# Mahdi-Si/VAE-TEB

Hardware: AMD Instinct MI355X
Metric: train samples/sec + ELBO, 4096-pt windows, batch 256, 1/2/4/8 MI355X (higher is better)
Workload: dtype bf16 MFMA (decoder heads + conv blocks + ResidualMLP linears, LSTM recurrences f16 fwd / bf16 bwd), fp32 accumulation; fp32 LayerNorm / BatchNorm / LSTM state / front-end / optimizer

## Files before the change

include/vaeteb.h:

```cpp
#ifndef VAETEB_H
#define VAETEB_H

#include <stdint.h>

#ifdef __cplusplus
extern "C" {
#endif

#define VT_OK 0
#define VT_ERR_ARG (-1)
#define VT_ERR_LAYOUT (-2)
#define VT_ERR_HIP (-3)

#define VT_FFT_MAX_LDS 8192

const char* vt_last_error(void);
int vt_stream_fork(void* from, void* to);
int vt_stream_mark(void* stream, int* slot);
int vt_stream_wait_mark(void* stream, int slot);
int vt_abi_version(void);
int vt_arrive_reset(void* stream);
int vt_capture_info(void* stream, char* buf, int len);
int vt_set_h16_format(int fp16);
int vt_get_h16_format(void);


int vt_fe_spectrum(const float* x, int64_t rows, int N, int n_pad, int pad_left, int pad_mode, const void* tw,
                   void* xhat, void* stream);

int vt_fe_lowpass(const float* x, int64_t rows, int64_t x_row_stride, int N, int n_pad, int pad_left,
                  const float* h0, int radius, int step, int start, int S, float* out, int64_t out_row_stride,
                  void* stream);

int vt_fe_wavelet(const void* xhat, int64_t B, int C, int n_pad, const float* psi, int n_items, const int* items,
                  const void* tw, int N, int pad_left, void* analytic, int n_slots, const float* h0, int radius,
                  int step, int start, int S, float* s1, int s1_channels, void* stream);

int vt_fe_pairs(const void* analytic, int64_t B, int n_slots, int N, int n_pad, int pad_left, int n_pairs,
                const int* slot_i, const int* slot_j, const float* power, const void* tw, const float* phi0, int dec,
                int start, int S, int pad_mode, float* out, void* stream);

int vt_fe_set_pairs_persist(int grid);
int vt_fe_set_pairs_direct(int on);
int vt_fe_set_pairs_half(int on);
int vt_fe_set_analytic_polar(int on);

int vt_fe_set_pairs_stamps(void* buf);

int vt_fe_normalize(const float* in, int64_t B, int C, int in_C, int S, const int* kind, const float* mean, const float* stdv,
                    float log_eps, float* out, int out_C, int out_off, void* stream);
int vt_fe_normalize_window(const float* in, int64_t B, int C, int in_C, int in_S, int s0, int S_len,
                           const int* kind, const float* mean, const float* stdv, float log_eps, float* out,
                           int out_C, int out_off, void* stream);
int vt_copy_cols(const float* src, int64_t rows, int ld_src, int src_col0, int ncols, float* dst, int ld_dst,
                 int dst_col0, void* stream);
int vt_clamp_bwd(const float* g, const float* x, int64_t n, float lo, float hi, float* gx, void* stream);
int vt_zero_ranges(float* base, int n, const int64_t* starts, const int64_t* ends, void* stream);
int vt_normalize_raw(const float* x, int64_t rows, int64_t row_stride, int N, float mean, float stdv, float* out,
                     void* stream);

#define VT_STATS_CHUNK_ROWS 32
#define VT_STATS_CHUNK_COLS 1024
int vt_stats_chunking(int* rows, int* cols);
int vt_stats_workspace_bytes(int64_t B, int C, int S_len, int64_t* bytes);
int vt_stats_accum(const float* in, int64_t B, int C, int in_C, int in_S, int s0, int S_len, const int* kind,
                   double log_eps, int64_t* count, double* sum, double* sum_sq, void* work, int64_t work_bytes,
                   void* stream);
int vt_stats_accum_raw(const float* x, int64_t rows, int64_t row_stride, int N, int64_t* count, double* sum,
                       double* sum_sq, void* work, int64_t work_bytes, void* stream);

int vt_fft(const void* in, void* out, int64_t rows, int n, int inverse, const void* tw, int tw_stride,
           void* stream);
int vt_fft_large(const void* in, void* out, void* ws, int64_t rows, int n, int inverse, const void* tw,
                 void* stream);
int vt_cdgmm(const void* A, const void* B, int b_is_real, void* C, int64_t rows, int n, void* stream);
int vt_scat_filter_sub(const void* A, int B, int64_t a_rows, int n, const int* a_idx, const float* pool,
                       const int64_t* f_off, int P, int k, void* out, void* stream);
int vt_scat_mod_spec(const void* A, int B, int64_t a_rows, int n, const int* a_idx, const float* pool,
                     const int64_t* f_off, int P, int k, const void* tw, void* out, void* stream);
int vt_scat_lowpass(const void* U, int B, int P, int n, const float* phi, int k, int i0, int i1, const int* ch,
                    int out_C, const void* tw, float* out, void* stream);
int vt_modulus_cplx(const void* in, void* out, int64_t count, void* stream);
int vt_modulus(const void* in, float* out, int64_t count, void* stream);
int vt_modulus_bwd(const void* in, const float* mod, const float* grad, void* grad_in, int64_t count, void* stream);
int vt_subsample_fourier(const void* in, void* out, int64_t rows, int n, int k, void* stream);
int vt_pad_reflect(const float* in, float* out, int64_t rows, int N, int pad_left, int pad_right, void* stream);


int vt_elbo_workspace_floats(void);

int vt_elbo_latent_fwd(const float* mu_c, const float* lv_q, const float* mu_y, const float* lv_p, const float* eps,
                       int64_t rows, int D, float* z, float* mu_post, float* kl, float* ws, void* stream);
int vt_elbo_latent_bwd(const float* mu_c, const float* lv_q, const float* mu_y, const float* lv_p, const float* eps,
                       int64_t rows, int D, const float* g_z, const float* g_mu_post, const float* g_kl,
                       float* g_mu_c, float* g_lv_q, float* g_mu_y, float* g_lv_p, void* stream);
int vt_elbo_output_fwd(const float* mu, const float* lv, const float* y, int64_t n_nll, const float* lin,
                       const float* t_st, const float* t_ph, int64_t rows, int c_st, int c_ph, float* g_mu,
                       float* g_lv, float* g_lin, float* nll, float* mse, float* ws, void* stream);
int vt_scale_by_device_scalar(float* x, int64_t n, const float* s, void* stream);

int vt_grad_norm_workspace_floats(void);
int vt_grad_norm_clip(const float* g, int64_t n, float pre_scale, float max_norm, float* out2, float* ws,
                      void* stream);
int vt_grad_norm_clip_scaled(const float* g, int64_t n, float pre_scale, float max_norm, float* out3, float* ws,
                             float* scaler, float growth_factor, float backoff_factor, int growth_interval,
                             void* stream);
int vt_adamw_step(float* p, const float* g, float* m, float* v, int64_t n, float lr, float beta1, float beta2,
                  float eps, float weight_decay, int step, const float* gscale, void* stream);
int vt_adamw_step_dev(float* p, const float* g, float* m, float* v, int64_t n, float lr, float beta1, float beta2,
                      float eps, float weight_decay, int* step, float* coef, const float* gscale, void* stream);
int vt_adamw_step_dev_shadow(float* p, const float* g, float* m, float* v, int64_t n, float lr, float beta1,
                             float beta2, float eps, float weight_decay, int* step, float* coef, const float* gscale,
                             int n_tiled, const int64_t* tiled_off, const int* tiled_N, const int* tiled_K,
                             const int64_t* tiled_w16, const int64_t* tiled_w16t, void* stream);
int vt_adamw_step_dev_skip(float* p, const float* g, float* m, float* v, int64_t n, float lr, float beta1,
                           float beta2, float eps, float weight_decay, int* step, float* coef, const float* gscale,
                           const float* skip, void* stream);
int vt_adamw_step_dev_shadow_skip(float* p, const float* g, float* m, float* v, int64_t n, float lr, float beta1,
                                  float beta2, float eps, float weight_decay, int* step, float* coef,
                                  const float* gscale, int n_tiled, const int64_t* tiled_off, const int* tiled_N,
                                  const int* tiled_K, const int64_t* tiled_w16, const int64_t* tiled_w16t,
                                  const float* skip, void* stream);
int vt_adamw_set_vector(int on);
int vt_cast_bf16(const float* src, void* dst, int64_t n, void* stream);
int vt_cast_bf16_to_f32(const void* src, float* dst, int64_t n, void* stream);

int vt_gemm_splits_hint(int64_t M, int N, int64_t K);
int vt_linear_fwd(const float* X, int64_t R, int K, const float* W, int N, const float* bias, float* Y, void* stream);
int vt_linear_bwd_data(const float* dY, int64_t R, int N, const float* W, int K, float* dX, int accumulate,
                       void* stream);
int vt_linear_bwd_weight(const float* dY, int64_t R, int N, const float* X, int K, float* dW, float* db,
                         int accumulate, float* ws, int64_t ws_floats, void* stream);
int vt_linear_ln_fwd(const float* X, int64_t R, int K, const float* W, int N, const float* bias, const float* gamma,
                     const float* beta, int act, float eps, float* Y, float* xhat, float* rstd, void* stream);
int vt_colsum(const float* X, int64_t R, int N, float* out, int accumulate, float* ws, int64_t ws_floats,
              void* stream);

#define VT_MLP_MAX_LAYERS 34
#define VT_MLP_MAX_WIDTH 144
int vt_resmlp_sizes(int n_layers, const int* dims, const int* layer_ln, const int* layer_act, int skip,
                    int64_t rows, int64_t* sizes);
int vt_resmlp_fwd(int n_layers, const int* dims, const int* layer_ln, const int* layer_act, int skip, float eps,
                  const float* const* params, const float* x, int64_t rows, float* out, float* xhat, float* rstd,
                  void* stream);
int vt_resmlp_bwd(int n_layers, const int* dims, const int* layer_ln, const int* layer_act, int skip, float eps,
                  const float* const* params, const float* dout, const float* xhat, const float* rstd, int64_t rows,
                  float* dx, float* const* grads, int accumulate, float* ws, int64_t ws_floats, void* stream);

int vt_resmlp_bf16_sizes(int n_layers, const int* dims, const int* layer_ln, const int* layer_act, int skip,
                         int64_t rows, int64_t* sizes);
int vt_resmlp_bf16_fwd(int n_layers, const int* dims, const int* layer_ln, const int* layer_act, int skip, float eps,
                       const float* const* params, const float* x, int64_t rows, float* out, float* xhat, float* rstd,
                       void* stream);
int vt_resmlp_bf16_bwd(int n_layers, const int* dims, const int* layer_ln, const int* layer_act, int skip, float eps,
                       const float* const* params, const float* dout, const float* xhat, const float* rstd,
                       int64_t rows, float* dx, float* const* grads, int accumulate, float* ws, int64_t ws_floats,
                       void* stream);
int vt_resmlp_bf16_plan(int n_layers, const int* dims, const int* layer_ln, const int* layer_act, int skip, float eps,
                        const float* const* params, int64_t rows, int64_t* handle, void* stream);
int vt_resmlp_bf16_prep_batch(int n, const int64_t* handles, void* stream);
int vt_resmlp_bf16_fwd_prepped(int n_layers, const int* dims, const int* layer_ln, const int* layer_act, int skip,
                               float eps, const float* const* params, const float* x, int64_t rows, float* out,
                               float* xhat, float* rstd, void* stream);
int vt_resmlp_bf16_split_sizes(int n_layers, const int* dims, const int* layer_ln, const int* layer_act, int skip,
                               int64_t rows, int64_t* sizes);
int vt_resmlp_bf16_bwd_data(int n_layers, const int* dims, const int* layer_ln, const int* layer_act, int skip,
                            float eps, const float* const* params, const float* dout, const float* xhat,
                            const float* rstd, int64_t rows, float* dx, float* const* grads, int accumulate,
                            void* dz16, float* ws, int64_t ws_floats, void* stream);
int vt_resmlp_bf16_bwd_weight(int n_layers, const int* dims, const int* layer_ln, const int* layer_act, int skip,
                              float eps, const float* const* params, const float* xhat, const void* dz16,
                              int64_t rows, float* const* grads, int accumulate, float* ws, int64_t ws_floats,
                              void* stream);
int vt_resmlp_bf16_set_stamps(void* buf);

int vt_mfma_supported(int K, int N);
int vt_mfma_workspace_floats(int64_t R, int K, int N, int64_t* floats);
int vt_mfma_weight_shadow(const float* W, int N, int K, void* W16, void* W16t, void* stream);
int vt_mfma_linear_fwd(const float* X, int64_t R, int K, const void* W16, int N, const float* bias, float* Y,
                       float* ws, int64_t ws_floats, void* stream);
int vt_mfma_linear_bwd_data(const float* dY, int64_t R, int N, const void* W16t, int K, float* dX, int accumulate,
                            float* ws, int64_t ws_floats, void* stream);
int vt_mfma_linear_bwd_weight(const float* dY, int64_t R, int N, const float* X, int K, float* dW, float* db,
                              int accumulate, float* ws, int64_t ws_floats, void* stream);

int vt_conv1d_out_len(int L_in, int K, int mode, int up);
int vt_conv1d_fwd(const float* X, int B, int L_in, int Cin, const float* W, int Cout, int K, int mode, int up,
                  float* Y, void* stream);
int vt_conv1d_bwd_data(const float* dY, int B, int L_in, int Cin, const float* W, int Cout, int K, int mode, int up,
                       float* dX, int accumulate, float* gpad, void* stream);
int vt_conv1d_bwd_weight(const float* dY, const float* X, int B, int L_in, int Cin, int Cout, int K, int mode, int up,
                         float* dW, int accumulate, float* ws, int64_t ws_floats, void* stream);
int vt_conv1d_bn_workspace_floats(int B, int L_in, int Cin, int Cout, int K, int mode, int up, int64_t* floats);
int vt_conv1d_bn_fwd(const float* X, int B, int L_in, int Cin, const float* W, int Cout, int K, int mode, int up,
                     const float* gamma, const float* beta, int act, float eps, float momentum, float* conv_out,
                     float* Y, float* mean, float* rstd, float* run_mean, float* run_var, float* ws,
                     int64_t ws_floats, void* stream);
int vt_conv1d_bf16_shadow(const float* W, int Cout, int Cin, int K, void* w16, void* w16t, void* stream);
int vt_conv1d_bf16_shadow_batch(int n, const int64_t* W, const int* Cout, const int* Cin, const int* K,
                                const int64_t* w16, const int64_t* w16t, void* stream);
int vt_conv_bf16_set_staging(int mode);
int vt_conv_bf16_set_kernels(int flags);
int vt_conv1d_bn_fwd_bf16(const float* X, int B, int L_in, int Cin, const void* w16, int Cout, int K, int mode,
                          int up, const float* gamma, const float* beta, int act, float eps, float momentum,
                          float* conv_out, float* Y, float* mean, float* rstd, float* run_mean, float* run_var,
                          float* ws, int64_t ws_floats, void* stream);
int vt_conv1d_bn_fwd_bf16_in(const float* X, const float* in_mean, const float* in_rstd, const float* in_gamma,
                             const float* in_beta, int in_act, int B, int L_in, int Cin, const void* w16, int Cout,
                             int K, int mode, int up, const float* gamma, const float* beta, int act, float eps,
                             float momentum, float* conv_out, float* Y, float* mean, float* rstd, float* run_mean,
                             float* run_var, float* ws, int64_t ws_floats, void* stream);
int vt_conv1d_fwd_bf16(const float* X, int B, int L_in, int Cin, const void* w16, int Cout, int K, int mode, int up,
                       float* Y, void* stream);
int vt_conv1d_bwd_gpad_bf16(const float* dY, int B, int L_in, int Cin, const void* w16t, int Cout, int K, int mode,
                            int up, float* gpad, void* stream);
int vt_conv1d_bwd_weight_bf16(const float* dY, const float* X, int B, int L_in, int Cin, int Cout, int K, int mode,
                              int up, float* dW, int accumulate, float* ws, int64_t ws_floats, void* stream);
int vt_conv1d_bwd_gpad_bf16_bn(const float* dY, const float* Xc, const float* bnp, int act, int64_t M, int B,
                               int L_in, int Cin, const void* w16t, int Cout, int K, int mode, int up, float* gpad,
                               void* dxbn16, void* stream);
int vt_conv1d_bwd_dx_bf16_bn(const float* dY, const float* Xc, const float* bnp, int act, int64_t M, int B, int L_in,
                             int Cin, const void* w16t, int Cout, int K, int mode, int up, float* dX, float* edge,
                             void* dxbn16, void* stream);
int vt_conv1d_bwd_weight_bf16_dy16(const void* dY16, const float* X, int B, int L_in, int Cin, int Cout, int K,
                                   int mode, int up, float* dW, int accumulate, float* ws, int64_t ws_floats,
                                   void* stream);
int vt_conv1d_bwd_weight_bf16_dy16s(const void* dY16, int dys, const float* X, int B, int L_in, int Cin, int Cout,
                                    int K, int mode, int up, float* dW, int accumulate, float* ws, int64_t ws_floats,
                                    void* stream);
int vt_conv1d_bwd_weight_bf16_in(const float* dY, const void* dY16, int dys, const float* X, const float* in_mean,
                                 const float* in_rstd, const float* in_gamma, const float* in_beta, int in_act, int B,
                                 int L_in, int Cin, int Cout, int K, int mode, int up, float* dW, int accumulate,
                                 float* ws, int64_t ws_floats, void* stream);
int vt_batchnorm_bwd_x16(const float* dY, const float* Xc, const float* bnp, int act, int64_t M, int C, void* d16,
                         void* stream);
int vt_conv1d_bwd_dx16(const void* d16, int B, int L_in, int Cin, const void* w16t, int Cout, int K, int mode, int up,
                       float* dX, float* edge, void* stream);
int vt_conv1d_direct_fwd(const float* X, int B, int L_in, int Cin, const float* W, int Cout, int K, int mode, int up,
                         float* Y, void* stream);
int vt_conv1d_direct_bwd_gpad(const float* dY, int B, int L_in, int Cin, const float* W, int Cout, int K, int mode,
                              int up, float* gpad, void* stream);
int vt_conv1d_fold(const float* gpad, int B, int L_in, int Cin, int Cout, int K, int mode, int up, float* dX,
                   int accumulate, void* stream);
int vt_conv1d_direct_bwd_weight(const float* dY, const float* X, int B, int L_in, int Cin, int Cout, int K, int mode,
                                int up, float* dW, int accumulate, float* ws, int64_t ws_floats, void* stream);

int vt_layernorm_fwd(const float* x, int64_t R, int C, const float* gamma, const float* beta, int act, float eps,
                     float* y, float* xhat, float* rstd, void* stream);
int vt_layernorm_bwd(const float* dy, const float* xhat, const float* rstd, int64_t R, int C, const float* gamma,
                     const float* beta, int act, float* dx, float* dgamma, float* dbeta, int accumulate_params,
                     float* ws, int64_t ws_floats, void* stream);
int vt_batchnorm_fwd(const float* x, int64_t M, int C, const float* gamma, const float* beta, int act, float eps,
                     float momentum, float* y, float* mean, float* rstd, float* run_mean, float* run_var, float* ws,
                     int64_t ws_floats, void* stream);
int vt_batchnorm_bwd(const float* dy, const float* x, int64_t M, int C, const float* mean, const float* rstd,
                     const float* gamma, const float* beta, int act, float* dx, float* dgamma, float* dbeta,
                     int accumulate_params, float* ws, int64_t ws_floats, void* stream);
int vt_batchnorm_fwd_dropout(const float* x, int64_t M, int C, const float* gamma, const float* beta, int act,
                             float eps, float momentum, float* y, float* mean, float* rstd, float* run_mean,
                             float* run_var, int L, float p, int64_t seed, const void* seed_offset, float* ws,
                             int64_t ws_floats, void* stream);
int vt_batchnorm_bwd_dropout(const float* dy, const float* x, int64_t M, int C, const float* mean, const float* rstd,
                             const float* gamma, const float* beta, int act, int L, float p, int64_t seed,
                             const void* seed_offset, float* dx, float* dgamma, float* dbeta, int accumulate_params,
                             float* ws, int64_t ws_floats, void* stream);
int vt_batchnorm_bwd_coef(const float* dy, const float* x, int64_t M, int C, const float* mean, const float* rstd,
                          const float* gamma, const float* beta, int act, float* dgamma, float* dbeta,
                          int accumulate_params, float* bnp, float* ws, int64_t ws_floats, void* stream);
int vt_batchnorm_eval(const float* x, int64_t M, int C, const float* run_mean, const float* run_var, float eps,
                      const float* gamma, const float* beta, int act, float* y, void* stream);
int vt_syncbn_sums(const float* x, const float* dy, int64_t M, int C, int which, const float* mean,
                   const float* rstd, const float* gamma, const float* beta, int act, double* sums, float* ws,
                   int64_t ws_floats, void* stream);
int vt_syncbn_stats(const double* sums, int C, int which, float eps, float momentum, float* mean, float* rstd,
                    float* run_mean, float* run_var, float* dgamma, float* dbeta, int accumulate, void* stream);
int vt_batchnorm_apply(const float* x, int64_t M, int C, const float* mean, const float* rstd, const float* gamma,
                       const float* beta, int act, float* y, void* stream);
int vt_syncbn_bwd_dx(const float* dy, const float* x, int64_t M, int C, const float* mean, const float* rstd,
                     const float* gamma, const float* beta, int act, const double* sums, float* dx, float* ws,
                     void* stream);
int vt_act_fwd(const float* x, int64_t n, int act, float* y, void* stream);
int vt_act_bwd(const float* dy, const float* x, int64_t n, int act, float* dx, void* stream);

int vt_lstm_layer_fwd(const float* gin, const float* w_hh, const float* b_hh, int B, int S, int hidden, float* out_h,
                      float* out_hprev, float* out_c, float* gates, void* stream);
int vt_lstm_layer_bwd(const float* dh_out, const float* gates, const float* cst, const float* w_hh, int B, int S,
                      int hidden, float* dgates, void* stream);
int vt_lstm_layer_fwd_x(const float* x, int In, const float* w_ih, const float* b_ih, const float* w_hh,
                        const float* b_hh, int B, int S, int hidden, float* out_h, float* out_hprev, float* out_c,
                        float* gates, void* stream);
int vt_lstm_layer_bwd_x(const float* dh_out, const float* gates, const float* cst, const float* w_hh,
                        const float* w_ih, int In, int B, int S, int hidden, float* dgates, float* dx, void* stream);
int vt_lstm16_layer_fwd(const float* x, int In, const float* w_ih, const float* b_ih, const float* w_hh,
                        const float* b_hh, int B, int S, int hidden, float* out_h, float* out_hprev, float* out_c,
                        float* gates, void* stream);
int vt_lstm16_layer_bwd(const float* dh_out, const float* gates, const float* cst, const float* w_hh,
                        const float* w_ih, int In, int B, int S, int hidden, float* dgates, float* dx, void* stream);
int vt_lstm16_pair_fwd(const float* x, int In, const float* w_ih0, const float* b_ih0, const float* w_hh0,
                       const float* b_hh0, const float* w_ih1, const float* b_ih1, const float* w_hh1,
                       const float* b_hh1, int B, int seq, int hidden, float* h0, float* c0, float* gates0, float* h1,
                       float* c1, float* gates1, void* stream);
int vt_lstm16_pair_bwd(const float* dh_out, const float* gates1, const float* c1, const float* w_hh1,
                       const float* w_ih1, const float* gates0, const float* c0, const float* w_hh0,
                       const float* w_ih0, int In0, int B, int seq, int hidden, void* dgates1, void* dgates0,
                       float* dx, void* stream, int dg_bf16);
int vt_lstm16_quad_fwd(const float* x, int In, const float* const* params, int B, int seq, int hidden,
                       float* const* outs, void* stream);
int vt_lstm16_quad_bwd(const float* dh_out, const float* const* w, const float* const* gc, int In0, int B, int seq,
                       int hidden, void* const* dg, float* dmid, float* dx, void* stream, int dg_bf16);
int vt_lstm16_chain_errors(int* count, int reset);
int vt_lstm_layer_bwd_weight(const float* dgates, const float* x, int In, const float* hprev, int B, int S,
                             int hidden, float* dw_ih, float* dw_hh, float* db_ih, float* db_hh, int accumulate,
                             float* ws, int64_t ws_floats, void* stream);
int vt_lstm16_layer_bwd_weight(const float* dgates, const float* x, int In, const float* h, int B, int S,
                               int hidden, float* dw_ih, float* dw_hh, float* db_ih, float* db_hh, int accumulate,
                               float* ws, int64_t ws_floats, void* stream);
int vt_lstm16_dg16_ok(int In);
int vt_lstm16_bwd_weight_multi(int nl, const void* const* dgates, const int* dg_bf16, const float* const* x,
                               const int* In, const float* const* h, int B, int seq, int hidden, float* const* grads,
                               const int* accumulate, float* ws, int64_t ws_floats, void* stream);

int vt_zconv_fwd(const float* X, int ldx, int B, int L, int Cin, const float* W, int Cout, int K, int pad_left,
                 float* Y, int ldy, int accumulate, void* stream);
int vt_zconv_bwd_data(const float* dY, int ldy, int B, int L, int Cin, const float* W, int Cout, int K, int pad_left,
                      float* dX, int ldx, int accumulate, void* stream);
int vt_zconv16_ws_floats(int Cin, int Cout, int K, int64_t* floats);
int vt_zconv16_fwd(const float* X, int ldx, int B, int L, int Cin, const float* W, int Cout, int K, int pad_left,
                   float* Y, int ldy, int accumulate, float* ws, int64_t ws_floats, void* stream);
int vt_zconv16_bwd_data(const float* dY, int ldy, int B, int L, int Cin, const float* W, int Cout, int K, int pad_left,
                        float* dX, int ldx, int accumulate, float* ws, int64_t ws_floats, void* stream);
int vt_zconv16_taps_elems(int Cin, int Cout, int K, int64_t* elems);
int vt_zconv16_taps(int n, const int64_t* W, const int* Cin, const int* Cout, const int* K, int flip,
                    const int64_t* T, void* stream);
int vt_zconv16_fwd_t(const float* X, int ldx, int B, int L, int Cin, const void* T, int Cout, int K, int pad_left,
                     float* Y, int ldy, int accumulate, void* stream);
int vt_zconv16_bwd_data_t(const float* dY, int ldy, int B, int L, int Cin, const void* T, int Cout, int K,
                          int pad_left, float* dX, int ldx, int accumulate, void* stream);
int vt_zconv16_bwd_weight(const float* dY, int ldy, const float* X, int ldx, int B, int L, int Cin, int Cout, int K,
                          int pad_left, float* dW, int accumulate, float* ws, int64_t ws_floats, void* stream);
int vt_zconv_bwd_weight_ws_floats(int B, int Cin, int Cout, int K, int64_t* floats);
int vt_zconv_bwd_weight(const float* dY, int ldy, const float* X, int ldx, int B, int L, int Cin, int Cout, int K,
                        int pad_left, float* dW, int accumulate, float* ws, int64_t ws_floats, void* stream);
int vt_maxpool3_fwd(const float* X, int B, int L, int C, float* Y, void* stream);
int vt_maxpool3_bwd(const float* dY, const float* X, int B, int L, int C, float* dX, int accumulate, void* stream);
int vt_add_act_fwd(const float* A, const float* Bm, int64_t n, int act, float* Y, void* stream);
int vt_add_act_dropout_fwd(const float* A, const float* Bm, int64_t n, int C, int act, int L, float p, int64_t seed,
                           const void* seed_offset, float* S_out, float* Y, void* stream);
int vt_act_dropout_bwd(const float* dY, const float* S_in, int64_t n, int C, int act, int L, float p, int64_t seed,
                       const void* seed_offset, float* dX, void* stream);
int vt_dropout_apply(const float* X, int64_t n, int C, int L, float p, int64_t seed, const void* seed_offset, float* Y,
                     void* stream);
int vt_dropout_seed_advance(void* offset, void* stream);
int vt_time_mean_fwd(const float* X, int B, int L, int C, float* Y, void* stream);
int vt_time_mean_bwd(const float* dY, int B, int L, int C, float* dX, int accumulate, void* stream);
int vt_attn_fwd(const float* qkv, int B, int S, int H, float scale, float p, int64_t seed, const void* seed_offset,
                float* out, float* lse, void* stream);
int vt_attn_bwd(const float* qkv, const float* out, const float* dout, const float* lse, int B, int S, int H,
                float scale, float p, int64_t seed, const void* seed_offset, float* dqkv, void* stream);
int vt_cross_entropy_fwd(const float* logits, const int64_t* labels, int B, int C, float* loss, float* probs,
                         void* stream);
int vt_cross_entropy_bwd(const float* probs, const int64_t* labels, int B, int C, const float* g, float* dlogits,
                         void* stream);

int vt_stepgraph_build(void* graph, int n_streams, void** handle);
int vt_stepgraph_launch(void* handle, void* const* streams);
int vt_stepgraph_info(void* handle, int* n_kernel, int* n_memcpy, int* n_memset, int* n_waits);
int vt_stepgraph_destroy(void* handle);
int vt_bucket_marker(int bucket, void* stream);
int vt_stepgraph_markers(void* handle, int* n_ops, int* n_markers, int* ends, int* buckets, int cap);
int vt_stepgraph_launch_range(void* handle, void* const* streams, int begin, int end, int flags);

#ifdef __cplusplus
}
#endif
#endif
```

vae-teb_amd/csrc/mfma.hip:

```cpp
#include "h16.h"

namespace vt {

constexpr int QM = 256, QN = 64, QK = 64, QT = 512;
constexpr int ROWB = QK * 2;
constexpr int A_BYTES = QM * ROWB;
constexpr int B_BYTES = QN * ROWB;
constexpr int NA = 3, NB = 8;
constexpr int GEMM_LDS = NA * A_BYTES + NB * B_BYTES;

__device__ __forceinline__ int swz(int r, int c) { return c ^ ((r >> 1) & 7); }

__device__ __forceinline__ void glds16(const void* src, char* lds) {
    __builtin_amdgcn_global_load_lds((const __attribute__((address_space(1))) void*)src,
                                     (__attribute__((address_space(3))) void*)lds, 16, 0, 0);
}

VT_ARRIVE_POOL(g_arrive_gemm);

typedef unsigned u32x4 __attribute__((ext_vector_type(4)));
__device__ __forceinline__ void st_agent4(__amdgpu_buffer_rsrc_t r, unsigned off, f32x4 v) {
    __builtin_amdgcn_raw_buffer_store_b128(__builtin_bit_cast(u32x4, v), r, (int)off, 0, CPOL_SC1);
}
__device__ __forceinline__ f32x4 ld_agent4(__amdgpu_buffer_rsrc_t r, unsigned off) {
    return __builtin_bit_cast(f32x4, __builtin_amdgcn_raw_buffer_load_b128(r, (int)off, 0, CPOL_SC1));
}

__device__ __forceinline__ bool last_arrival_in(unsigned* ctr, unsigned total, unsigned* flag) {
    asm volatile("s_waitcnt vmcnt(0)" ::: "memory");
    __syncthreads();
    if (threadIdx.x == 0) {
        const unsigned old = atomicAdd(ctr, 1u);
        const bool last = old == total - 1;
        if (last) atomicExch(ctr, 0u);
        *flag = last ? 1u : 0u;
    }
    __syncthreads();
    return *flag != 0u;
}

template <typename H>
__global__ __launch_bounds__(QT) void k_mfma_gemm(const H* __restrict__ A, int64_t lda,
                                                  const H* __restrict__ B, int64_t ldb, int M, int N, int K,
                                                  float* __restrict__ C, int64_t ldc, const float* __restrict__ bias,
                                                  int accumulate, float* __restrict__ part, unsigned slot0) {
    extern __shared__ __attribute__((aligned(16))) char smem[];
    char* sa = smem;
    char* sb = smem + NA * A_BYTES;
    const int tid = threadIdx.x, lane = tid & 63, w = tid >> 6;
    const int n0 = blockIdx.x * QN, m0 = blockIdx.y * QM;
    const int64_t kbeg = (int64_t)blockIdx.z * K;
    const int T = K / QK;

    const int rsub = lane >> 3, pos = lane & 7;
    auto kof = [&](int t) { return kbeg + (int64_t)(t < T ? t : T - 1) * QK; };
    auto issue_a = [&](int t) {
        const int64_t k0 = kof(t);
        char* st = sa + (t % NA) * A_BYTES;
#pragma unroll
        for (int i = 0; i < 4; ++i) {
            const int r = 32 * w + 8 * i + rsub;
            glds16(A + (int64_t)(m0 + r) * lda + k0 + 8 * swz(r, pos), st + (32 * w + 8 * i) * ROWB);
        }
    };
    auto issue_b = [&](int t) {
        const int64_t k0 = kof(t);
        const int r = 8 * w + rsub;
        glds16(B + (int64_t)(n0 + r) * ldb + k0 + 8 * swz(r, pos), sb + (t % NB) * B_BYTES + 8 * w * ROWB);
    };

    f32x4 acc[2][4];
#pragma unroll
    for (int i = 0; i < 2; ++i)
#pragma unroll
        for (int j = 0; j < 4; ++j) acc[i][j] = f32x4{0.f, 0.f, 0.f, 0.f};

    const int lr = lane & 15, lc = lane >> 4;
    auto compute = [&](int t) {
        const char* ta = sa + (t % NA) * A_BYTES;
        const char* tb = sb + (t % NB) * B_BYTES;
#pragma unroll
        for (int h = 0; h < 2; ++h) {
            const int c = 4 * h + lc;
            hv8<H> af[2], bfr[4];
#pragma unroll
            for (int i = 0; i < 2; ++i) {
                const int r = 32 * w + 16 * i + lr;
                af[i] = *(const hv8<H>*)(ta + r * ROWB + 16 * swz(r, c));
            }
#pragma unroll
            for (int j = 0; j < 4; ++j) {
                const int r = 16 * j + lr;
                bfr[j] = *(const hv8<H>*)(tb + r * ROWB + 16 * swz(r, c));
            }
#pragma unroll
            for (int i = 0; i < 2; ++i)
#pragma unroll
                for (int j = 0; j < 4; ++j)
                    acc[i][j] = mfma16(af[i], bfr[j], acc[i][j]);
        }
    };

#pragma unroll
    for (int t = 0; t < NB - 1; ++t) issue_b(t);
    issue_a(0);
    issue_a(1);
    for (int t = 0; t < T; ++t) {
        if (t == 0) asm volatile("s_waitcnt vmcnt(4)" ::: "memory");
        else if (t == 1) asm volatile("s_waitcnt vmcnt(5)" ::: "memory");
        else asm volatile("s_waitcnt vmcnt(6)" ::: "memory");
        asm volatile("s_waitcnt lgkmcnt(0)" ::: "memory");
        __builtin_amdgcn_s_barrier();
        issue_a(t + 2);
        issue_b(t + NB - 1);
        compute(t);
    }
    asm volatile("s_waitcnt vmcnt(0)" ::: "memory");

    if (part) {
        const int splits = gridDim.z, z = blockIdx.z;
        const unsigned tile = blockIdx.y * gridDim.x + blockIdx.x;
        const int64_t slab = (int64_t)QT * 32 * 4;
        const __amdgpu_buffer_rsrc_t pr = agent_rsrc(part + (int64_t)tile * splits * QT * 32, splits * slab);
#pragma unroll
        for (int g = 0; g < 8; ++g) st_agent4(pr, (unsigned)(z * slab + (g * QT + tid) * 16), acc[g >> 2][g & 3]);
        if (!last_arrival_in(&g_arrive_gemm[slot0 + tile], (unsigned)splits, (unsigned*)smem)) return;
#pragma unroll
        for (int g = 0; g < 8; ++g) {
            f32x4 s = z == 0 ? acc[g >> 2][g & 3] : ld_agent4(pr, (unsigned)((g * QT + tid) * 16));
            for (int p = 1; p < splits; ++p)
                s += p == z ? acc[g >> 2][g & 3] : ld_agent4(pr, (unsigned)(p * slab + (g * QT + tid) * 16));
            acc[g >> 2][g & 3] = s;
        }
    }
#pragma unroll
    for (int i = 0; i < 2; ++i)
#pragma unroll
        for (int j = 0; j < 4; ++j) {
            const int col = n0 + 16 * j + lr;
            const float bcol = bias ? bias[col] : 0.f;
#pragma unroll
            for (int r = 0; r < 4; ++r) {
                const int row = m0 + 32 * w + 16 * i + 4 * lc + r;
                if (row >= M) continue;
                float o = acc[i][j][r] + bcol;
                if (accumulate) o = C[(int64_t)row * ldc + col] + o;
                C[(int64_t)row * ldc + col] = o;
            }
        }
}

template <typename H>
__global__ void k_bf16_rows(const float* __restrict__ X, int64_t M, int K, H* __restrict__ out, int64_t Mpad,
                            int Kpad) {
    const int64_t i = (int64_t)blockIdx.x * blockDim.x + threadIdx.x;
    const int64_t total = Mpad * Kpad;
    if (i >= total) return;
    const int64_t m = i / Kpad;
    const int k = (int)(i - m * Kpad);
    out[i] = (m < M && k < K) ? (H)X[m * K + k] : (H)0.f;
}

template <typename H>
__global__ __launch_bounds__(256) void k_bf16_transpose(const float* __restrict__ X, int64_t R, int Cn,
                                                        H* __restrict__ out, int64_t Cpad, int64_t Rpad) {
    __shared__ float tile[64][65];
    const int64_t r0 = (int64_t)blockIdx.x * 64, c0 = (int64_t)blockIdx.y * 64;
    const int tx = threadIdx.x & 63, ty = threadIdx.x >> 6;
    for (int i = ty; i < 64; i += 4) {
        const int64_t r = r0 + i, c = c0 + tx;
        tile[i][tx] = (r < R && c < Cn) ? X[r * Cn + c] : 0.f;
    }
    __syncthreads();
    for (int i = ty; i < 64; i += 4) {
        const int64_t c = c0 + i, r = r0 + tx;
        if (c < Cpad && r < Rpad) out[c * Rpad + r] = (H)tile[tx][i];
    }
}

template <typename H>
__global__ __launch_bounds__(256) void k_bf16_shadow(const float* __restrict__ W, int N, int K,
                                                     H* __restrict__ W16, H* __restrict__ W16t) {
    __shared__ float tile[64][65];
    const int64_t n0 = (int64_t)blockIdx.y * 64, k0 = (int64_t)blockIdx.x * 64;
    const int tx = threadIdx.x & 63, ty = threadIdx.x >> 6;
    for (int i = ty; i < 64; i += 4) {
        const float v = W[(n0 + i) * K + k0 + tx];
        tile[i][tx] = v;
        W16[(n0 + i) * K + k0 + tx] = (H)v;
    }
    __syncthreads();
    for (int i = ty; i < 64; i += 4) W16t[(k0 + i) * N + n0 + tx] = (H)tile[tx][i];
}

typedef short v4i16 __attribute__((ext_vector_type(4)));
typedef short v8i16 __attribute__((ext_vector_type(8)));
constexpr int DWT = 128, DWC = 64;
constexpr int DWS = DWT + 16;
constexpr int DWIMG = DWC * DWS + (DWC / 8) * 64;

__device__ __forceinline__ int dw_pos(int r, int c) { return r * DWS + (r >> 3) * 64 + c; }

template <typename H>
__device__ __forceinline__ hv8<H> dw_frag(const H* img, int row0, int col0) {
    const int lane = threadIdx.x & 63, g = lane >> 4, q = (lane >> 2) & 3, p = lane & 3;
    const H* a0 = img + dw_pos(row0 + 8 * g + q, col0 + 4 * p);
    const H* a1 = img + dw_pos(row0 + 8 * g + q + 4, col0 + 4 * p);
    const v4i16 lo = __builtin_amdgcn_ds_read_tr16_b64_v4i16((__attribute__((address_space(3))) v4i16*)a0);
    const v4i16 hi = __builtin_amdgcn_ds_read_tr16_b64_v4i16((__attribute__((address_space(3))) v4i16*)a1);
    const v8i16 r = __builtin_shufflevector(lo, hi, 0, 1, 2, 3, 4, 5, 6, 7);
    return __builtin_bit_cast(hv8<H>, r);
}

template <typename H>
__global__ __launch_bounds__(256) void k_mfma_dw(const float* __restrict__ dY, int64_t R, int N,
                                                 const float* __restrict__ X, int K, float* __restrict__ dW,
                                                 int accumulate) {
    __shared__ __attribute__((aligned(16))) H img[2][DWIMG];
    const int tid = threadIdx.x, lane = tid & 63, w = tid >> 6, wm = w >> 1, wn = w & 1;
    const int n0 = blockIdx.y * DWT, k0 = blockIdx.x * DWT;
    float4 pf[2][8];
    auto load = [&](int64_t r0) {
#pragma unroll
        for (int i = 0; i < 8; ++i) {
            const int e = tid + 256 * i, row = e >> 5, q4 = e & 31;
            const bool ok = r0 + row < R;
            pf[0][i] = ok ? *(const float4*)(dY + (r0 + row) * N + n0 + 4 * q4) : make_float4(0.f, 0.f, 0.f, 0.f);
            pf[1][i] = ok ? *(const float4*)(X + (r0 + row) * K + k0 + 4 * q4) : make_float4(0.f, 0.f, 0.f, 0.f);
        }
    };
    auto store = [&]() {
#pragma unroll
        for (int o = 0; o < 2; ++o)
#pragma unroll
            for (int i = 0; i < 8; ++i) {
                const int e = tid + 256 * i, row = e >> 5, q4 = e & 31;
                const hv4<H> v = {(H)pf[o][i].x, (H)pf[o][i].y, (H)pf[o][i].z, (H)pf[o][i].w};
                *(hv4<H>*)(img[o] + dw_pos(row, 4 * q4)) = v;
            }
    };
    f32x4 acc[4][4];
#pragma unroll
    for (int i = 0; i < 4; ++i)
#pragma unroll
        for (int j = 0; j < 4; ++j) acc[i][j] = f32x4{0.f, 0.f, 0.f, 0.f};
    load(0);
    for (int64_t r0 = 0; r0 < R; r0 += DWC) {
        store();
        __syncthreads();
        if (r0 + DWC < R) load(r0 + DWC);
#pragma unroll
        for (int s = 0; s < DWC / 32; ++s) {
            hv8<H> a[4], b[4];
#pragma unroll
            for (int i = 0; i < 4; ++i) a[i] = dw_frag(img[0], 32 * s, 64 * wm + 16 * i);
#pragma unroll
            for (int j = 0; j < 4; ++j) b[j] = dw_frag(img[1], 32 * s, 64 * wn + 16 * j);
#pragma unroll
            for (int i = 0; i < 4; ++i)
#pragma unroll
                for (int j = 0; j < 4; ++j)
                    acc[i][j] = mfma16(a[i], b[j], acc[i][j]);
        }
        __syncthreads();
    }
    const int lr = lane & 15, lc = lane >> 4;
    float* c0 = dW + (int64_t)(n0 + 64 * wm + 4 * lc) * K + k0 + 64 * wn + lr;
    if (accumulate) {
        f32x4 old[4][4];
#pragma unroll
        for (int i = 0; i < 4; ++i)
#pragma unroll
            for (int j = 0; j < 4; ++j)
#pragma unroll
                for (int rr = 0; rr < 4; ++rr) old[i][j][rr] = c0[(int64_t)(16 * i + rr) * K + 16 * j];
#pragma unroll
        for (int i = 0; i < 4; ++i)
#pragma unroll
            for (int j = 0; j < 4; ++j) acc[i][j] += old[i][j];
    }
#pragma unroll
    for (int i = 0; i < 4; ++i)
#pragma unroll
        for (int j = 0; j < 4; ++j)
#pragma unroll
            for (int rr = 0; rr < 4; ++rr) c0[(int64_t)(16 * i + rr) * K + 16 * j] = acc[i][j][rr];
}

static inline int64_t up_to(int64_t x, int64_t m) { return (x + m - 1) / m * m; }

static int mfma_splits(int64_t tiles, int64_t ktiles) {
    int best = 1;
    for (int64_t d = 1; d <= ktiles && d <= 64; ++d)
        if (ktiles % d == 0 && tiles * d <= 320) best = (int)d;
    return best;
}

struct MfmaPlan {
    int64_t Mpad, Kpad, a_floats, part_floats;
    int splits;
};

static MfmaPlan plan(int64_t M, int N, int64_t K) {
    MfmaPlan p;
    p.Mpad = up_to(M, QM);
    p.Kpad = up_to(K, QK);
    p.a_floats = up_to(p.Mpad * p.Kpad / 2, 64);
    p.splits = mfma_splits((p.Mpad / QM) * (N / QN), p.Kpad / QK);
    p.part_floats = p.splits > 1 ? (int64_t)p.splits * p.Mpad * N : 0;
    return p;
}

template <typename H>
static int run(const char* who, const H* A, const H* B, int64_t ldb, int64_t M, int N, const MfmaPlan& p,
               float* C, const float* bias, int accumulate, float* part, hipStream_t st) {
    static bool attr = false;
    if (!attr) {
        if (hipFuncSetAttribute((const void*)k_mfma_gemm<H>, hipFuncAttributeMaxDynamicSharedMemorySize, GEMM_LDS) !=
            hipSuccess) {
            set_error("%s: cannot allow %d B of LDS for k_mfma_gemm", who, GEMM_LDS);
            return VT_ERR_HIP;
        }
        attr = true;
    }
    const int kper = (int)(p.Kpad / p.splits);
    dim3 grid(N / QN, (unsigned)(p.Mpad / QM), p.splits);
    const unsigned tiles = grid.x * grid.y;
    hipLaunchKernelGGL(k_mfma_gemm<H>, grid, dim3(QT), GEMM_LDS, st, A, p.Kpad, B, ldb, (int)M, N, kper, C, (int64_t)N,
                       bias, accumulate, p.splits > 1 ? part : nullptr, p.splits > 1 ? arrive_slots(tiles, st) : 0u);
    VT_LAUNCH_CHECK(who);
    return VT_OK;
}

}

using namespace vt;

extern "C" {

int vt_mfma_supported(int K, int N) { return (K > 0 && N > 0 && K % QK == 0 && N % QN == 0) ? 1 : 0; }

int vt_mfma_workspace_floats(int64_t R, int K, int N, int64_t* floats) {
    VT_CHECK_ARG(R > 0 && K > 0 && N > 0 && floats, "vt_mfma_workspace_floats: shape");
    MfmaPlan f = plan(R, N, K), d = plan(R, K, N), w = plan(N, K, R);
    const int64_t wf = w.a_floats + up_to((int64_t)K * w.Kpad / 2, 64) + w.part_floats + N;
    int64_t m = f.a_floats + f.part_floats;
    if (d.a_floats + d.part_floats > m) m = d.a_floats + d.part_floats;
    if (wf > m) m = wf;
    *floats = m;
    return VT_OK;
}

int vt_mfma_weight_shadow(const float* W, int N, int K, void* W16, void* W16t, void* stream) {
    VT_CHECK_ARG(vt_mfma_supported(K, N) && W && W16 && W16t, "vt_mfma_weight_shadow: K and N must be multiples of 64");
    VT_H16(hipLaunchKernelGGL(k_bf16_shadow<H>, dim3(K / 64, N / 64), dim3(256), 0, S(stream), W, N, K, (H*)W16,
                              (H*)W16t));
    VT_LAUNCH_CHECK("vt_mfma_weight_shadow");
    return VT_OK;
}

int vt_mfma_linear_fwd(const float* X, int64_t R, int K, const void* W16, int N, const float* bias, float* Y,
                       float* ws, int64_t ws_floats, void* stream) {
    VT_CHECK_ARG(R > 0 && vt_mfma_supported(K, N), "vt_mfma_linear_fwd: K and N must be positive multiples of 64");
    MfmaPlan p = plan(R, N, K);
    VT_CHECK_ARG(p.a_floats + p.part_floats <= ws_floats, "vt_mfma_linear_fwd: workspace too small");
    const int64_t tot = p.Mpad * p.Kpad;
    int rc = VT_OK;
    VT_H16(H* A = (H*)ws;
           hipLaunchKernelGGL(k_bf16_rows<H>, dim3((unsigned)((tot + 255) / 256)), dim3(256), 0, S(stream), X, R, K, A,
                              p.Mpad, (int)p.Kpad);
           rc = run("vt_mfma_linear_fwd", (const H*)A, (const H*)W16, K, R, N, p, Y, bias, 0, ws + p.a_floats,
                    S(stream)));
    return rc;
}

int vt_mfma_linear_bwd_data(const float* dY, int64_t R, int N, const void* W16t, int K, float* dX, int accumulate,
                            float* ws, int64_t ws_floats, void* stream) {
    VT_CHECK_ARG(R > 0 && vt_mfma_supported(N, K), "vt_mfma_linear_bwd_data: K and N must be positive multiples of 64");
    MfmaPlan p = plan(R, K, N);
    VT_CHECK_ARG(p.a_floats + p.part_floats <= ws_floats, "vt_mfma_linear_bwd_data: workspace too small");
    const int64_t tot = p.Mpad * p.Kpad;
    int rc = VT_OK;
    VT_H16(H* A = (H*)ws;
           hipLaunchKernelGGL(k_bf16_rows<H>, dim3((unsigned)((tot + 255) / 256)), dim3(256), 0, S(stream), dY, R, N, A,
                              p.Mpad, (int)p.Kpad);
           rc = run("vt_mfma_linear_bwd_data", (const H*)A, (const H*)W16t, N, R, K, p, dX, nullptr, accumulate,
                    ws + p.a_floats, S(stream)));
    return rc;
}

int vt_mfma_linear_bwd_weight(const float* dY, int64_t R, int N, const float* X, int K, float* dW, float* db,
                              int accumulate, float* ws, int64_t ws_floats, void* stream) {
    VT_CHECK_ARG(R > 0 && vt_mfma_supported(K, N), "vt_mfma_linear_bwd_weight: K and N must be positive multiples of 64");
    if (N % DWT == 0 && K % DWT == 0) {
        VT_H16(hipLaunchKernelGGL(k_mfma_dw<H>, dim3(K / DWT, N / DWT), dim3(256), 0, S(stream), dY, R, N, X, K, dW,
                                  accumulate));
        VT_LAUNCH_CHECK("vt_mfma_linear_bwd_weight");
        return db ? vt_colsum(dY, R, N, db, accumulate, ws, ws_floats, stream) : VT_OK;
    }
    MfmaPlan p = plan(N, K, R);
    const int64_t b_floats = up_to((int64_t)K * p.Kpad / 2, 64);
    VT_CHECK_ARG(p.a_floats + b_floats + p.part_floats + N <= ws_floats, "vt_mfma_linear_bwd_weight: workspace too small");
    float* part = ws + p.a_floats + b_floats;
    int rc = VT_OK;
    VT_H16(H* A = (H*)ws;
           H* Bt = (H*)(ws + p.a_floats);
           hipLaunchKernelGGL(k_bf16_transpose<H>, dim3((unsigned)(p.Kpad / 64), (unsigned)(p.Mpad / 64)), dim3(256), 0,
                              S(stream), dY, R, N, A, p.Mpad, p.Kpad);
           hipLaunchKernelGGL(k_bf16_transpose<H>, dim3((unsigned)(p.Kpad / 64), (unsigned)(K / 64)), dim3(256), 0,
                              S(stream), X, R, K, Bt, (int64_t)K, p.Kpad);
           rc = run("vt_mfma_linear_bwd_weight", (const H*)A, (const H*)Bt, p.Kpad, N, K, p, dW, nullptr, accumulate,
                    part, S(stream)));
    if (rc || !db) return rc;
    return vt_colsum(dY, R, N, db, accumulate, part, ws_floats - p.a_floats - b_floats, stream);
}

}
```

Before: 33830.

## Add in-workgroup split-K MFMA GEMM for linear forward and backward-data

Adds a new GEMM kernel in which the four wave pairs of a 512-thread workgroup each handle one quarter of K on a 64x64 output tile. The partial sums are then reduced through LDS and written with the bias, instead of using the old 256-row tile with grid-level split-K partial buffers. The planner selects it by default for forward and data-gradient linears when padded K is a multiple of 256. The aim is more workgroups for small-M or skinny GEMMs and no extra partial-sum global traffic or reduction pass. A toggle restores the old grid-split path.

```diff
diff --git a/include/vaeteb.h b/include/vaeteb.h
--- a/include/vaeteb.h
+++ b/include/vaeteb.h
@@ -183,6 +183,7 @@
                             float* ws, int64_t ws_floats, void* stream);
 int vt_mfma_linear_bwd_weight(const float* dY, int64_t R, int N, const float* X, int K, float* dW, float* db,
                               int accumulate, float* ws, int64_t ws_floats, void* stream);
+int vt_mfma_set_grid_split(int on);
 
 int vt_conv1d_out_len(int L_in, int K, int mode, int up);
 int vt_conv1d_fwd(const float* X, int B, int L_in, int Cin, const float* W, int Cout, int K, int mode, int up,
diff --git a/vae-teb_amd/csrc/mfma.hip b/vae-teb_amd/csrc/mfma.hip
--- a/vae-teb_amd/csrc/mfma.hip
+++ b/vae-teb_amd/csrc/mfma.hip
@@ -150,6 +150,126 @@
         }
 }
 
+constexpr int WM = 64;
+constexpr int WQ_BYTES = WM * ROWB;
+constexpr int W_STAGE = 4 * WQ_BYTES;
+constexpr int WNA = 2, WNB = 3;
+constexpr int WG_LDS = (WNA + WNB) * W_STAGE;
+constexpr int WP_ROW = QN + 4;
+static_assert(WNA == 2 && WNB >= WNA, "k_mfma_gemm_wg: the vmcnt derivation assumes A one tile ahead, B at least as far");
+static_assert(WG_LDS <= 160 * 1024 && 4 * WM * WP_ROW * 4 <= WG_LDS, "k_mfma_gemm_wg: LDS budget");
+
+template <typename H>
+__global__ __launch_bounds__(QT) void k_mfma_gemm_wg(const H* __restrict__ A, int64_t lda,
+                                                     const H* __restrict__ B, int64_t ldb, int M, int N, int K,
+                                                     float* __restrict__ C, int64_t ldc,
+                                                     const float* __restrict__ bias, int accumulate) {
+    extern __shared__ __attribute__((aligned(16))) char smem[];
+    char* sa = smem;
+    char* sb = smem + WNA * W_STAGE;
+    const int tid = threadIdx.x, lane = tid & 63, w = tid >> 6, q = w >> 1, hm = w & 1;
+    const int n0 = blockIdx.x * QN, m0 = blockIdx.y * WM;
+    const int64_t kbeg = (int64_t)q * K;
+    const int T = K / QK;
+
+    const int rsub = lane >> 3, pos = lane & 7;
+    auto issue = [&](const H* src, int64_t ld, int row0, char* stages, int nst, int t) {
+        if (t < 0 || t >= T) return;
+        const int64_t k0 = kbeg + (int64_t)t * QK;
+        char* st = stages + (t % nst) * W_STAGE + q * WQ_BYTES;
+#pragma unroll
+        for (int i = 0; i < 4; ++i) {
+            const int r = 32 * hm + 8 * i + rsub;
+            glds16(src + (int64_t)(row0 + r) * ld + k0 + 8 * swz(r, pos), st + (32 * hm + 8 * i) * ROWB);
+        }
+    };
+    auto issue_a = [&](int t) { issue(A, lda, m0, sa, WNA, t); };
+    auto issue_b = [&](int t) { issue(B, ldb, n0, sb, WNB, t); };
+
+    f32x4 acc[2][4];
+#pragma unroll
+    for (int i = 0; i < 2; ++i)
+#pragma unroll
+        for (int j = 0; j < 4; ++j) acc[i][j] = f32x4{0.f, 0.f, 0.f, 0.f};
+
+    const int lr = lane & 15, lc = lane >> 4;
+    auto compute = [&](int t) {
+        const char* ta = sa + (t % WNA) * W_STAGE + q * WQ_BYTES;
+        const char* tb = sb + (t % WNB) * W_STAGE + q * WQ_BYTES;
+#pragma unroll
+        for (int h = 0; h < 2; ++h) {
+            const int c = 4 * h + lc;
+            hv8<H> af[2], bfr[4];
+#pragma unroll
+            for (int i = 0; i < 2; ++i) {
+                const int r = 32 * hm + 16 * i + lr;
+                af[i] = *(const hv8<H>*)(ta + r * ROWB + 16 * swz(r, c));
+            }
+#pragma unroll
+            for (int j = 0; j < 4; ++j) {
+                const int r = 16 * j + lr;
+                bfr[j] = *(const hv8<H>*)(tb + r * ROWB + 16 * swz(r, c));
+            }
+#pragma unroll
+            for (int i = 0; i < 2; ++i)
+#pragma unroll
+                for (int j = 0; j < 4; ++j)
+                    acc[i][j] = mfma16(af[i], bfr[j], acc[i][j]);
+        }
+    };
+
+#pragma unroll
+    for (int t = 0; t < WNB - WNA; ++t) issue_b(t);
+#pragma unroll
+    for (int s = 1 - WNA; s < 0; ++s) {
+        issue_a(s + WNA - 1);
+        issue_b(s + WNB - 1);
+    }
+    for (int t = 0; t < T; ++t) {
+        if (WNB > WNA && t + WNB - WNA < T) asm volatile("s_waitcnt vmcnt(4)" ::: "memory");
+        else asm volatile("s_waitcnt vmcnt(0)" ::: "memory");
+        asm volatile("s_waitcnt lgkmcnt(0)" ::: "memory");
+        __builtin_amdgcn_s_barrier();
+        issue_a(t + WNA - 1);
+        issue_b(t + WNB - 1);
+        compute(t);
+    }
+    asm volatile("s_waitcnt lgkmcnt(0)" ::: "memory");
+    __builtin_amdgcn_s_barrier();
+
+    float* pp = (float*)smem;
+#pragma unroll
+    for (int i = 0; i < 2; ++i)
+#pragma unroll
+        for (int j = 0; j < 4; ++j)
+#pragma unroll
+            for (int r = 0; r < 4; ++r)
+                pp[(q * WM + 32 * hm + 16 * i + 4 * lc + r) * WP_ROW + 16 * j + lr] = acc[i][j][r];
+    __syncthreads();
+    const int col = n0 + 4 * (tid & 15);
+    f32x4 bv = f32x4{0.f, 0.f, 0.f, 0.f};
+    if (bias) bv = f32x4{bias[col], bias[col + 1], bias[col + 2], bias[col + 3]};
+    const bool vec = (((uintptr_t)C | (uintptr_t)(ldc * 4)) & 15) == 0;
+#pragma unroll
+    for (int g = 0; g < 2; ++g) {
+        const int tr = (tid >> 4) + 32 * g, row = m0 + tr;
+        if (row >= M) continue;
+        const float* p0 = pp + tr * WP_ROW + 4 * (tid & 15);
+        f32x4 s = *(const f32x4*)p0;
+#pragma unroll
+        for (int p = 1; p < 4; ++p) s += *(const f32x4*)(p0 + p * WM * WP_ROW);
+        f32x4 o = s + bv;
+        float* c = C + (int64_t)row * ldc + col;
+        if (vec) {
+            if (accumulate) o = *(const f32x4*)c + o;
+            *(f32x4*)c = o;
+        } else {
+#pragma unroll
+            for (int e = 0; e < 4; ++e) c[e] = accumulate ? c[e] + o[e] : o[e];
+        }
+    }
+}
+
 template <typename H>
 __global__ void k_bf16_rows(const float* __restrict__ X, int64_t M, int K, H* __restrict__ out, int64_t Mpad,
                             int Kpad) {
@@ -299,21 +419,45 @@
 struct MfmaPlan {
     int64_t Mpad, Kpad, a_floats, part_floats;
     int splits;
+    bool wg;
 };
 
-static MfmaPlan plan(int64_t M, int N, int64_t K) {
+static int g_mfma_grid_split = 0;
+
+static MfmaPlan plan(int64_t M, int N, int64_t K, bool may_wg) {
     MfmaPlan p;
-    p.Mpad = up_to(M, QM);
     p.Kpad = up_to(K, QK);
+    p.wg = may_wg && !g_mfma_grid_split && p.Kpad % (4 * QK) == 0 &&
+           up_to(M, WM) / WM <= 65535;
+    p.Mpad = up_to(M, p.wg ? WM : QM);
     p.a_floats = up_to(p.Mpad * p.Kpad / 2, 64);
-    p.splits = mfma_splits((p.Mpad / QM) * (N / QN), p.Kpad / QK);
-    p.part_floats = p.splits > 1 ? (int64_t)p.splits * p.Mpad * N : 0;
+    p.splits = p.wg ? 4 : mfma_splits((p.Mpad / QM) * (N / QN), p.Kpad / QK);
+    p.part_floats = !p.wg && p.splits > 1 ? (int64_t)p.splits * p.Mpad * N : 0;
     return p;
+}
+
+template <typename H>
+static int run_wg(const char* who, const H* A, const H* B, int64_t ldb, int64_t M, int N, const MfmaPlan& p,
+                  float* C, const float* bias, int accumulate, hipStream_t st) {
+    static bool attr = false;
+    if (!attr) {
+        if (hipFuncSetAttribute((const void*)k_mfma_gemm_wg<H>, hipFuncAttributeMaxDynamicSharedMemorySize, WG_LDS) !=
+            hipSuccess) {
+            set_error("%s: cannot allow %d B of LDS for k_mfma_gemm_wg", who, WG_LDS);
+            return VT_ERR_HIP;
+        }
+        attr = true;
+    }
+    hipLaunchKernelGGL(k_mfma_gemm_wg<H>, dim3(N / QN, (unsigned)(p.Mpad / WM)), dim3(QT), WG_LDS, st, A, p.Kpad, B, ldb,
+                       (int)M, N, (int)(p.Kpad / 4), C, (int64_t)N, bias, accumulate);
+    VT_LAUNCH_CHECK(who);
+    return VT_OK;
 }
 
 template <typename H>
 static int run(const char* who, const H* A, const H* B, int64_t ldb, int64_t M, int N, const MfmaPlan& p,
                float* C, const float* bias, int accumulate, float* part, hipStream_t st) {
+    if (p.wg) return run_wg(who, A, B, ldb, M, N, p, C, bias, accumulate, st);
     static bool attr = false;
     if (!attr) {
         if (hipFuncSetAttribute((const void*)k_mfma_gemm<H>, hipFuncAttributeMaxDynamicSharedMemorySize, GEMM_LDS) !=
@@ -342,7 +486,7 @@
 
 int vt_mfma_workspace_floats(int64_t R, int K, int N, int64_t* floats) {
     VT_CHECK_ARG(R > 0 && K > 0 && N > 0 && floats, "vt_mfma_workspace_floats: shape");
-    MfmaPlan f = plan(R, N, K), d = plan(R, K, N), w = plan(N, K, R);
+    MfmaPlan f = plan(R, N, K, true), d = plan(R, K, N, true), w = plan(N, K, R, false);
     const int64_t wf = w.a_floats + up_to((int64_t)K * w.Kpad / 2, 64) + w.part_floats + N;
     int64_t m = f.a_floats + f.part_floats;
     if (d.a_floats + d.part_floats > m) m = d.a_floats + d.part_floats;
@@ -362,7 +506,7 @@
 int vt_mfma_linear_fwd(const float* X, int64_t R, int K, const void* W16, int N, const float* bias, float* Y,
                        float* ws, int64_t ws_floats, void* stream) {
     VT_CHECK_ARG(R > 0 && vt_mfma_supported(K, N), "vt_mfma_linear_fwd: K and N must be positive multiples of 64");
-    MfmaPlan p = plan(R, N, K);
+    MfmaPlan p = plan(R, N, K, true);
     VT_CHECK_ARG(p.a_floats + p.part_floats <= ws_floats, "vt_mfma_linear_fwd: workspace too small");
     const int64_t tot = p.Mpad * p.Kpad;
     int rc = VT_OK;
@@ -377,7 +521,7 @@
 int vt_mfma_linear_bwd_data(const float* dY, int64_t R, int N, const void* W16t, int K, float* dX, int accumulate,
                             float* ws, int64_t ws_floats, void* stream) {
     VT_CHECK_ARG(R > 0 && vt_mfma_supported(N, K), "vt_mfma_linear_bwd_data: K and N must be positive multiples of 64");
-    MfmaPlan p = plan(R, K, N);
+    MfmaPlan p = plan(R, K, N, true);
     VT_CHECK_ARG(p.a_floats + p.part_floats <= ws_floats, "vt_mfma_linear_bwd_data: workspace too small");
     const int64_t tot = p.Mpad * p.Kpad;
     int rc = VT_OK;
@@ -398,7 +542,7 @@
         VT_LAUNCH_CHECK("vt_mfma_linear_bwd_weight");
         return db ? vt_colsum(dY, R, N, db, accumulate, ws, ws_floats, stream) : VT_OK;
     }
-    MfmaPlan p = plan(N, K, R);
+    MfmaPlan p = plan(N, K, R, false);
     const int64_t b_floats = up_to((int64_t)K * p.Kpad / 2, 64);
     VT_CHECK_ARG(p.a_floats + b_floats + p.part_floats + N <= ws_floats, "vt_mfma_linear_bwd_weight: workspace too small");
     float* part = ws + p.a_floats + b_floats;
@@ -415,4 +559,9 @@
     return vt_colsum(dY, R, N, db, accumulate, part, ws_floats - p.a_floats - b_floats, stream);
 }
 
-}
+int vt_mfma_set_grid_split(int on) {
+    g_mfma_grid_split = on ? 1 : 0;
+    return VT_OK;
+}
+
+}
```

After: 34040, median of 6. Within noise of the previous version (+0.6%).
